# aconz2/font-ocr

Measured on AMD Instinct MI355X. Metric: Mpixels/s scanned (95-glyph x --x-bits=2 bank), higher is better.
Workload: dtype i8

## Files before the change

font_ocr_amd/csrc/hip/post.hip:

```cpp
#include <cstring>

#include "common.h"

namespace focr {

__device__ __forceinline__ int32_t total_key(float f) {
    int32_t b = __float_as_int(f);
    return b ^ (int32_t)(((uint32_t)(b >> 31)) >> 1);
}

__global__ void mark_anchor_rows(const uint64_t *__restrict__ hkeys, const float *__restrict__ hsims, const uint8_t *__restrict__ keep,
                                 const uint64_t *__restrict__ n_p, uint64_t ub, KeyFmt fmt, float anchor, uint32_t r_h, uint8_t *__restrict__ keep_row,
                                 uint32_t *__restrict__ line_b, uint32_t *__restrict__ line_e) {
    size_t i = (size_t)blockIdx.x * blockDim.x + threadIdx.x;
    const size_t n = (size_t)min(*n_p, ub);
    if (i >= n) return;
    const uint64_t k = hkeys[i];
    const size_t row = (size_t)fmt.page(k) * r_h + fmt.y(k);
    if (i == 0 || fmt.line(hkeys[i - 1]) != fmt.line(k)) line_b[row] = (uint32_t)i;
    if (i + 1 == n || fmt.line(hkeys[i + 1]) != fmt.line(k)) line_e[row] = (uint32_t)(i + 1);
    if (keep[i] && hsims[i] >= anchor) keep_row[row] = 1;
}

__device__ __forceinline__ uint32_t wave_umax(uint32_t v) {
    v = max(v, (uint32_t)__builtin_amdgcn_update_dpp(0, (int)v, 0x111, 0xf, 0xf, true));
    v = max(v, (uint32_t)__builtin_amdgcn_update_dpp(0, (int)v, 0x112, 0xf, 0xf, true));
    v = max(v, (uint32_t)__builtin_amdgcn_update_dpp(0, (int)v, 0x114, 0xf, 0xf, true));
    v = max(v, (uint32_t)__builtin_amdgcn_update_dpp(0, (int)v, 0x118, 0xf, 0xf, true));
    v = max(v, (uint32_t)__builtin_amdgcn_update_dpp(0, (int)v, 0x142, 0xa, 0xf, true));
    v = max(v, (uint32_t)__builtin_amdgcn_update_dpp(0, (int)v, 0x143, 0xc, 0xf, true));
    return (uint32_t)__builtin_amdgcn_readlane((int)v, 63);
}

constexpr uint32_t WALK_ROWS = 16;

struct Top {
    uint32_t ord, idx, letter, t, x;
    bool has;
};
__device__ __forceinline__ bool top_beats(const Top &a, const Top &b) { return b.has && (!a.has || b.ord > a.ord || (b.ord == a.ord && b.idx > a.idx)); }
struct RunnerArgs {
    const uint32_t *t_letter;
    const uint64_t *scanned;
    focr_runner_t *out;
    uint32_t bound;
};
__device__ __forceinline__ void store_runner(const RunnerArgs &ra, uint32_t slot, uint32_t members, const Top &second) {
    if (slot >= ra.bound) return;
    focr_runner_t r;
    r.members = members;
    r.letter = r.template_index = FOCR_NO_RUNNER;
    r.similarity = -__builtin_inff();
    r.x = r.reserved = 0;
    if (second.has) {
        r.letter = second.letter;
        r.template_index = second.t;
        r.similarity = __int_as_float(total_key(__int_as_float((int32_t)(second.ord ^ 0x80000000u))));
        r.x = (uint16_t)second.x;
    }
    ra.out[slot] = r;
}

struct NoArgs {};
__device__ __forceinline__ NoArgs runner_args() { return {}; }
__device__ __forceinline__ const RunnerArgs &runner_args(const RunnerArgs &ra) { return ra; }
template <bool RUNNERS, typename... Extra>
__global__ __launch_bounds__(256) void walk_kernel(const uint64_t *__restrict__ keys, const float *__restrict__ sims,
                                                   const uint8_t *__restrict__ keep, KeyFmt fmt, uint32_t n_rows_total,
                                                   int32_t overlap, const uint8_t *__restrict__ keep_row,
                                                   const uint32_t *__restrict__ line_b, const uint32_t *__restrict__ line_e,
                                                   uint32_t *__restrict__ choice, uint64_t *__restrict__ row_groups,
                                                   const Extra... extra) {
    static_assert(sizeof...(Extra) == (RUNNERS ? 1 : 0), "walk_runners takes one RunnerArgs, walk_lines nothing");
    [[maybe_unused]] const auto ra = runner_args(extra...);
    const uint32_t wave_id = (blockIdx.x * blockDim.x + threadIdx.x) >> 6, lane = threadIdx.x & 63;
    const uint32_t row_first = wave_id * WALK_ROWS;
    if (row_first >= n_rows_total) return;
    const uint32_t my_row = row_first + lane;
    const bool mine = lane < WALK_ROWS && my_row < n_rows_total && keep_row[my_row] != 0;
    const uint32_t my_b = mine ? line_b[my_row] : 0u, my_e = mine ? line_e[my_row] : 0u;
    for (uint64_t todo = __builtin_amdgcn_ballot_w64(mine); todo; todo &= todo - 1) {
    const int src = (int)__builtin_ctzll(todo);
    const uint32_t wave = row_first + (uint32_t)src;
    const uint64_t b = (uint32_t)__builtin_amdgcn_readlane((int)my_b, src), e = (uint32_t)__builtin_amdgcn_readlane((int)my_e, src);

    uint32_t groups = 0;
    bool open = false;
    int32_t anchor = 0;
    uint32_t best_ord = 0, best_idx = 0;
    Top a1{}, a2{};
    uint32_t members = 0, slot0 = 0;
    if constexpr (RUNNERS) slot0 = (uint32_t)ra.scanned[wave];
    for (uint64_t base = b; base < e; base += 64) {
        const uint64_t i = base + lane;
        const bool valid = i < e && keep[i];
        const int32_t x = valid ? (int32_t)fmt.x(keys[i]) : 0x7fffffff;
        const uint32_t ord = valid ? ((uint32_t)total_key(sims[i]) ^ 0x80000000u) : 0u;
        uint32_t let = 0, tt = 0;
        if constexpr (RUNNERS) {
            tt = valid ? fmt.t(keys[i]) : 0u;
            let = valid ? ra.t_letter[tt] : 0u;
        }
        const uint64_t vmask = __builtin_amdgcn_ballot_w64(valid);
        uint32_t pos = 0;
        int32_t opened_at = -1;
        while (pos < 64) {
            if (!open) {
                const uint64_t cand = vmask & (~0ull << pos);
                if (!cand) break;
                pos = (uint32_t)__builtin_ctzll(cand);
                anchor = __builtin_amdgcn_readlane(x, (int)pos);
                opened_at = (int32_t)pos;
                best_ord = 0;
                best_idx = 0;
                open = true;
                if constexpr (RUNNERS) a1.has = a2.has = false, members = 0;
            }
            const bool in = valid && lane >= pos && ((int32_t)lane == opened_at || ((x - anchor <= overlap) && (anchor - x <= overlap)));
            const uint64_t inmask = __builtin_amdgcn_ballot_w64(in);
            const uint64_t brk = vmask & ~inmask & (~0ull << pos);
            const uint32_t stop = brk ? (uint32_t)__builtin_ctzll(brk) : 64u;
            const bool member = in && lane < stop;
            const uint32_t mx = wave_umax(member ? ord : 0u);
            const uint64_t top = __builtin_amdgcn_ballot_w64(member && ord == mx);
            if (top && mx >= best_ord) {
                best_ord = mx;
                best_idx = (uint32_t)(base - b) + (63u - (uint32_t)__builtin_clzll(top));
            }
            if constexpr (RUNNERS) {
                members += (uint32_t)__builtin_popcountll(__builtin_amdgcn_ballot_w64(member));
                if (top) {
                    const int l1 = 63 - (int)__builtin_clzll(top);
                    const Top m1{mx, (uint32_t)(base - b) + (uint32_t)l1, (uint32_t)__builtin_amdgcn_readlane((int)let, l1),
                                 (uint32_t)__builtin_amdgcn_readlane((int)tt, l1), (uint32_t)__builtin_amdgcn_readlane(x, l1), true};
                    Top m2{};
                    const bool other = member && let != m1.letter;
                    if (__builtin_amdgcn_ballot_w64(other)) {
                        const uint32_t mx2 = wave_umax(other ? ord : 0u);
                        const int l2 = 63 - (int)__builtin_clzll(__builtin_amdgcn_ballot_w64(other && ord == mx2));
                        m2 = Top{mx2, (uint32_t)(base - b) + (uint32_t)l2, (uint32_t)__builtin_amdgcn_readlane((int)let, l2),
                                 (uint32_t)__builtin_amdgcn_readlane((int)tt, l2), (uint32_t)__builtin_amdgcn_readlane(x, l2), true};
                    }
                    Top lose = m1;
                    if (!a1.has || m1.ord >= a1.ord) lose = a1, a1 = m1;
                    Top s{};
                    if (lose.has && lose.letter != a1.letter) s = lose;
                    if (a2.has && a2.letter != a1.letter && top_beats(s, a2)) s = a2;
                    if (m2.has && m2.letter != a1.letter && top_beats(s, m2)) s = m2;
                    a2 = s;
                }
            }
            if (stop < 64) {
                if constexpr (RUNNERS) {
                    if (lane == 0) store_runner(ra, slot0 + groups, members, a2);
                } else {
                    if (lane == 0) choice[b + groups] = (uint32_t)b + best_idx;
                }
                groups++;
                open = false;
            }
            pos = stop;
        }
    }
    if (open) {
        if constexpr (RUNNERS) {
            if (lane == 0) store_runner(ra, slot0 + groups, members, a2);
        } else {
            if (lane == 0) choice[b + groups] = (uint32_t)b + best_idx;
        }
        groups++;
    }
    if constexpr (!RUNNERS)
        if (lane == 0) row_groups[wave] = ((uint64_t)1 << 32) | groups;
    }
}

constexpr auto walk_lines = walk_kernel<false>;
constexpr auto walk_runners = walk_kernel<true, RunnerArgs>;

__global__ void emit_chars(const uint64_t *__restrict__ keys, const float *__restrict__ sims, const uint64_t *__restrict__ n_p, uint64_t ub, KeyFmt fmt, uint32_t r_h,
                           const uint8_t *__restrict__ keep_row, const uint32_t *__restrict__ line_b,
                           const uint32_t *__restrict__ choice, const uint64_t *__restrict__ row_groups,
                           const uint64_t *__restrict__ scanned, const uint32_t *__restrict__ t_w,
                           const uint32_t *__restrict__ t_h, const uint32_t *__restrict__ t_letter,
                           uint64_t *__restrict__ line_char_off, focr_hit_t *__restrict__ chars) {
    size_t i = (size_t)blockIdx.x * blockDim.x + threadIdx.x;
    if (i >= min(*n_p, ub)) return;
    const uint64_t ki = keys[i];
    const size_t row = (size_t)fmt.page(ki) * r_h + fmt.y(ki);
    if (!keep_row[row]) return;
    const uint32_t k = (uint32_t)i - line_b[row];
    if (k >= (uint32_t)row_groups[row]) return;
    const uint64_t sc = scanned[row];
    const uint64_t off = (sc & 0xffffffffu) + k;
    if (k == 0) line_char_off[sc >> 32] = sc & 0xffffffffu;
    const uint32_t e = choice[i];
    const uint64_t key = keys[e];
    const uint32_t t = fmt.t(key);
    focr_hit_t h;
    h.x = (uint16_t)fmt.x(key);
    h.y = (uint16_t)fmt.y(key);
    h.w = (uint16_t)t_w[t];
    h.h = (uint16_t)t_h[t];
    h.similarity = sims[e];
    h.letter = t_letter[t];
    h.template_index = t;
    chars[off] = h;
}

__global__ void page_offsets(const uint64_t *__restrict__ scanned, uint32_t r_h, uint32_t n_pages, uint64_t *__restrict__ page_line_off) {
    uint32_t p = blockIdx.x * blockDim.x + threadIdx.x;
    if (p > n_pages) return;
    page_line_off[p] = scanned[(size_t)min(p, n_pages) * r_h] >> 32;
}

__global__ __launch_bounds__(256) void copy_chars_kernel(const uint32_t *__restrict__ src, const uint64_t *__restrict__ total, uint32_t *__restrict__ dst, uint64_t dst_dwords) {
    constexpr uint64_t DW = sizeof(focr_hit_t) / 4;
    const uint64_t n = min((*total & 0xffffffffull) * DW, dst_dwords);
    for (uint64_t i = (uint64_t)blockIdx.x * blockDim.x + threadIdx.x; i < n; i += (uint64_t)gridDim.x * blockDim.x) dst[i] = src[i];
}

bool post_queue_chars_copy(focr_ctx *c, void *dst, size_t dst_bytes) {
    static_assert(sizeof(focr_hit_t) % 4 == 0, "focr_hit_t is copied as dwords");
    if (!c->post_pending || !c->post_scanned.p || !c->post_chars.p || !dst) return false;
    const size_t n_rows_total = c->n_pages * c->pages.r_h;
    hipLaunchKernelGGL(copy_chars_kernel, dim3(64), dim3(256), 0, c->stream, (const uint32_t *)c->post_chars.p, (const uint64_t *)c->post_scanned.p + n_rows_total,
                       (uint32_t *)dst, (uint64_t)(dst_bytes / 4));
    return hipGetLastError() == hipSuccess;
}

}

using namespace focr;

extern "C" {

int focr_process_hits(focr_ctx_t *c, float anchor_threshold, int32_t overlap) {
    if (!c) return FOCR_ERR_INVALID;
    if (!c->scanned) return fail(c, FOCR_ERR_STATE, "focr_process_hits: no scan results");
    FOCR_HIP(c, hipSetDevice(c->device));
    c->post_starts();
    c->post_anchor = anchor_threshold;
    c->post_overlap = overlap;
    const size_t ub = c->ub_hits, n_pages = c->n_pages;
    if (!c->sizes_pending && (c->n_hits == 0 || c->n_matches == 0)) {
        c->processed = true;
        c->ms[MS_POST] = 0.f;
        return FOCR_OK;
    }
    if (ub >= 0xffffffffull) return fail(c, FOCR_ERR_OVERFLOW, "focr_process_hits: more than 2^32 hits in one batch");
    FOCR_HIP(c, hipEventRecord(c->ev[EV_POST_BEGIN], c->stream));
    const size_t n_rows_total = n_pages * c->pages.r_h;
    if (!c->scratch(c->post_keep, n_rows_total + 8) || !c->scratch(c->post_choice, ub + 1) || !c->scratch(c->post_packed, n_rows_total + 1) ||
        !c->scratch(c->post_scanned, n_rows_total + 1) || !c->scratch(c->post_page_off, n_pages + 1) || !c->scratch(c->post_line_be, 2 * n_rows_total) ||
        !c->scratch(c->post_line_off, n_rows_total + 1) || !c->scratch(c->post_chars, ub + 1))
        return fail(c, FOCR_ERR_NOMEM, "focr_process_hits: hipMalloc failed");
    uint8_t *keep_row = c->post_keep;
    uint32_t *choice = c->post_choice, *line_b = c->post_line_be, *line_e = line_b + n_rows_total;
    uint64_t *packed = c->post_packed, *scanned = c->post_scanned;
    uint64_t *d_page_off = c->post_page_off, *d_line_off = c->post_line_off;
    focr_hit_t *d_chars = c->post_chars;
    const uint8_t *keep = c->ord_keep;
    {
        ClearList clear{};
        if (!clear.add(keep_row, n_rows_total)) return fail(c, FOCR_ERR_INVALID, "focr_process_hits: clear list full or region too large");
        if (!clear.add(packed, (n_rows_total + 1) * 8)) return fail(c, FOCR_ERR_INVALID, "focr_process_hits: clear list full or region too large");
        if (int rc = launch_clear(c, clear)) return rc;
    }
    const unsigned nb = (unsigned)((ub + 255) / 256);
    if (ub)
        hipLaunchKernelGGL(mark_anchor_rows, dim3(nb), dim3(256), 0, c->stream, c->d_hkeys, c->d_hsims, keep, c->d_n_hits, (uint64_t)ub, c->fmt,
                           anchor_threshold, (uint32_t)c->pages.r_h, keep_row, line_b, line_e);
    hipLaunchKernelGGL(walk_lines, dim3((unsigned)(((n_rows_total + WALK_ROWS - 1) / WALK_ROWS * 64 + 255) / 256)), dim3(256), 0, c->stream, c->d_hkeys, c->d_hsims,
                       keep, c->fmt, (uint32_t)n_rows_total, overlap, keep_row, line_b, line_e, choice, packed);
    int rc;
    if ((rc = exclusive_scan_u64(c, packed, scanned, n_rows_total + 1))) return rc;
    FOCR_HIP(c, hipMemcpyAsync(&c->h_res->lines_chars, scanned + n_rows_total, sizeof(uint64_t), hipMemcpyDeviceToHost, c->stream));
    if (ub)
        hipLaunchKernelGGL(emit_chars, dim3(nb), dim3(256), 0, c->stream, c->d_hkeys, c->d_hsims, c->d_n_hits, (uint64_t)ub, c->fmt, (uint32_t)c->pages.r_h,
                           keep_row, line_b, choice, packed, scanned, c->bank.d_t_w, c->bank.d_t_h, c->bank.d_t_letter, d_line_off, d_chars);
    hipLaunchKernelGGL(page_offsets, dim3((unsigned)((n_pages + 1 + 255) / 256)), dim3(256), 0, c->stream, scanned, (uint32_t)c->pages.r_h,
                       (uint32_t)n_pages, d_page_off);
    FOCR_HIP(c, hipGetLastError());
    FOCR_HIP(c, hipEventRecord(c->ev[EV_POST_END], c->stream));
    c->post_pending = true;
    c->processed = true;
    if (!c->sizes_pending) return finish_results(c);
    return FOCR_OK;
}

static int fetch_lines(focr_ctx *c) {
    int rc0 = finish_results(c);
    if (rc0) return rc0;
    if (c->lines_on_host) return FOCR_OK;
    c->h_page_line_off.assign(c->n_pages + 1, 0);
    c->h_line_char_off.assign(c->n_lines + 1, 0);
    c->h_chars.resize(c->n_chars);
    if (c->n_matches && (c->n_lines || c->n_chars)) {
        FOCR_HIP(c, hipSetDevice(c->device));
        if (c->n_lines)
            FOCR_HIP(c, hipMemcpyAsync(c->h_line_char_off.data(), c->post_line_off.p, c->n_lines * 8, hipMemcpyDeviceToHost, c->io_stream));
        FOCR_HIP(c, hipMemcpyAsync(c->h_page_line_off.data(), c->post_page_off.p, (c->n_pages + 1) * 8, hipMemcpyDeviceToHost, c->io_stream));
        if (c->n_chars)
            FOCR_HIP(c, hipMemcpyAsync(c->h_chars.data(), c->post_chars.p, c->n_chars * sizeof(focr_hit_t), hipMemcpyDeviceToHost, c->io_stream));
        FOCR_HIP(c, hipStreamSynchronize(c->io_stream));
    }
    c->h_line_char_off[c->n_lines] = c->n_chars;
    c->lines_on_host = true;
    return FOCR_OK;
}

size_t focr_total_chars(focr_ctx_t *c) { return (c && c->processed && finish_results(c) == FOCR_OK) ? c->n_chars : 0; }
size_t focr_total_lines(focr_ctx_t *c) { return (c && c->processed && finish_results(c) == FOCR_OK) ? c->n_lines : 0; }

int focr_get_lines(focr_ctx_t *c, uint64_t *page_line_offsets, uint64_t *line_char_offsets, focr_hit_t *chars) {
    if (!c) return FOCR_ERR_INVALID;
    if (!c->processed) return fail(c, FOCR_ERR_STATE, "focr_get_lines: call focr_process_hits first");
    int rc = fetch_lines(c);
    if (rc) return rc;
    if (page_line_offsets) memcpy(page_line_offsets, c->h_page_line_off.data(), c->h_page_line_off.size() * 8);
    if (line_char_offsets) memcpy(line_char_offsets, c->h_line_char_off.data(), c->h_line_char_off.size() * 8);
    if (chars && c->n_chars) memcpy(chars, c->h_chars.data(), c->n_chars * sizeof(focr_hit_t));
    return FOCR_OK;
}

int focr_get_lines_into(focr_ctx_t *c, uint64_t *page_line_offsets, uint64_t *line_char_offsets, focr_hit_t *chars) {
    if (!c || !page_line_offsets || !line_char_offsets || !chars) return FOCR_ERR_INVALID;
    if (!c->processed) return fail(c, FOCR_ERR_STATE, "focr_get_lines_into: call focr_process_hits first");
    int rc = finish_results(c);
    if (rc) return rc;
    FOCR_HIP(c, hipSetDevice(c->device));
    if (c->n_matches && (c->n_lines || c->n_chars)) {
        if (c->n_lines) FOCR_HIP(c, hipMemcpyAsync(line_char_offsets, c->post_line_off.p, c->n_lines * 8, hipMemcpyDeviceToHost, c->io_stream));
        FOCR_HIP(c, hipMemcpyAsync(page_line_offsets, c->post_page_off.p, (c->n_pages + 1) * 8, hipMemcpyDeviceToHost, c->io_stream));
        if (c->n_chars) FOCR_HIP(c, hipMemcpyAsync(chars, c->post_chars.p, c->n_chars * sizeof(focr_hit_t), hipMemcpyDeviceToHost, c->io_stream));
        FOCR_HIP(c, hipStreamSynchronize(c->io_stream));
    } else {
        for (size_t p = 0; p <= c->n_pages; p++) page_line_offsets[p] = 0;
    }
    line_char_offsets[c->n_lines] = c->n_chars;
    return FOCR_OK;
}

const focr_hit_t *focr_lines_device_chars(focr_ctx_t *c) {
    return (c && c->processed && finish_results(c) == FOCR_OK && c->n_chars) ? (const focr_hit_t *)c->post_chars.p : nullptr;
}

int focr_get_runners(focr_ctx_t *c, focr_runner_t *out) {
    if (!c) return FOCR_ERR_INVALID;
    c->run_ms = 0.f;
    c->run_launches = 0;
    if (!c->scanned || !c->processed) return fail(c, FOCR_ERR_STATE, "focr_get_runners: call focr_process_hits first (after the last scan)");
    if (int rc = finish_results(c)) return rc;
    const size_t n_chars = c->n_chars;
    if (!n_chars) return FOCR_OK;
    if (!out) return fail(c, FOCR_ERR_INVALID, "focr_get_runners: no output buffer");
    FOCR_HIP(c, hipSetDevice(c->device));
    const hipStream_t s = c->io_stream;
    if (!c->runners_valid) {
        const size_t bound = c->ub_hits + 1, n_rows_total = c->n_pages * c->pages.r_h;
        if (bound >= 0xffffffffull) return fail(c, FOCR_ERR_OVERFLOW, "focr_get_runners: more than 2^32 hits in one batch");
        if (c->post_runners.reserve(bound, Grow::quarter, nullptr) != hipSuccess) return fail(c, FOCR_ERR_NOMEM, "focr_get_runners: hipMalloc failed");
        FOCR_HIP(c, hipEventRecord(c->run_ev[0], s));
        hipLaunchKernelGGL(walk_runners, dim3((unsigned)(((n_rows_total + WALK_ROWS - 1) / WALK_ROWS * 64 + 255) / 256)), dim3(256), 0, s, (const uint64_t *)c->d_hkeys,
                           (const float *)c->d_hsims, (const uint8_t *)c->ord_keep.p, c->fmt, (uint32_t)n_rows_total, c->post_overlap, (const uint8_t *)c->post_keep.p,
                           (const uint32_t *)c->post_line_be.p, (const uint32_t *)c->post_line_be.p + n_rows_total, (uint32_t *)nullptr, (uint64_t *)nullptr,
                           RunnerArgs{c->bank.d_t_letter.p, c->post_scanned.p, c->post_runners.p, (uint32_t)bound});
        FOCR_HIP(c, hipGetLastError());
        FOCR_HIP(c, hipEventRecord(c->run_ev[1], s));
    }
    FOCR_HIP(c, hipMemcpyAsync(out, c->post_runners.p, n_chars * sizeof(focr_runner_t), hipMemcpyDeviceToHost, s));
    FOCR_HIP(c, hipStreamSynchronize(s));
    if (!c->runners_valid) {
        FOCR_HIP(c, hipEventElapsedTime(&c->run_ms, c->run_ev[0], c->run_ev[1]));
        c->run_launches = 1;
        c->runners_valid = true;
    }
    return FOCR_OK;
}

int focr_last_runners(focr_ctx_t *c, float *ms, uint32_t *launches) {
    if (!c) return FOCR_ERR_INVALID;
    if (ms) *ms = c->run_ms;
    if (launches) *launches = c->run_launches;
    return FOCR_OK;
}

int focr_debug_process_hits(focr_ctx_t *c, const uint32_t *page, const uint32_t *y, const uint32_t *x, const uint32_t *t,
                            const float *similarity, const uint8_t *keep, size_t n) {
    if (!c) return FOCR_ERR_INVALID;
    if (n && (!page || !y || !x || !t || !similarity || !keep)) return fail(c, FOCR_ERR_INVALID, "focr_debug_process_hits: bad arguments");
    if (!c->n_templates || !c->pages.u8) return fail(c, FOCR_ERR_STATE, "focr_debug_process_hits: upload a bank and allocate pages first");
    if (n >= 0xffffffffull) return fail(c, FOCR_ERR_OVERFLOW, "focr_debug_process_hits: more than 2^32 hits in one batch");
    const KeyFmt fmt = key_format(c->n_templates, c->pages.r_w, c->pages.r_h, c->n_pages);
    std::vector<uint64_t> keys(n);
    std::vector<uint8_t> kept(n);
    size_t n_kept = 0;
    for (size_t i = 0; i < n; i++) {
        if (page[i] >= c->n_pages || y[i] >= c->pages.r_h || x[i] >= c->pages.r_w || t[i] >= c->n_templates)
            return fail(c, FOCR_ERR_INVALID, "focr_debug_process_hits: hit " + std::to_string(i) + " lies outside the pages or the bank");
        keys[i] = fmt.pack(page[i], y[i], x[i], t[i]);
        if (i && keys[i] <= keys[i - 1])
            return fail(c, FOCR_ERR_INVALID, "focr_debug_process_hits: hit " + std::to_string(i) + " does not follow its predecessor in (page, y, x, t)");
        kept[i] = keep[i] != 0;
        n_kept += kept[i];
    }
    if (int rc = finish_results(c)) return rc;
    FOCR_HIP(c, hipSetDevice(c->device));
    if (!c->scratch(c->acc_hkeys, n + 1) || !c->scratch(c->acc_hsims, n + 1) || !c->scratch(c->ord_keep, n + 1))
        return fail(c, FOCR_ERR_NOMEM, "focr_debug_process_hits: hipMalloc failed");
    uint64_t *d_keys = c->acc_hkeys;
    float *d_sims = c->acc_hsims;
    uint8_t *d_keep = c->ord_keep;
    if (n) {
        FOCR_HIP(c, hipMemcpyAsync(d_keys, keys.data(), n * 8, hipMemcpyHostToDevice, c->stream));
        FOCR_HIP(c, hipMemcpyAsync(d_sims, similarity, n * 4, hipMemcpyHostToDevice, c->stream));
        FOCR_HIP(c, hipMemcpyAsync(d_keep, kept.data(), n, hipMemcpyHostToDevice, c->stream));
    }
    if (int rc = install_host_hits(c, n)) return rc;
    FOCR_HIP(c, hipStreamSynchronize(c->stream));
    c->fmt = fmt;
    c->d_hkeys = d_keys;
    c->d_hsims = d_sims;
    c->n_hits = c->n_hits_raw = n;
    c->n_matches = n_kept;
    c->sub_p0 = 0;
    c->sub_np = c->n_pages;
    c->estimated = false;
    c->debug_hits_installed();
    return FOCR_OK;
}

}
```

Baseline: 34200.

## Fuse anchor marking into row walk with binary search and parallel chunk walk

Drops the clear launch and the per-hit mark_anchor_rows kernel. A new walk_rows kernel binary-searches the sorted keys to find each 16-row window's hit range, computes line begin/end, the anchor flags and zeroed row_groups itself, then walks each row 64 hits at a time using wave-parallel jump pointers and segmented max scans instead of a serial scan. emit_chars becomes a row-parallel emit_rows kernel. This saves launches and memory passes over all hits, but the walk logic is much more intricate, which raises the risk of subtle grouping mismatches.

```diff
diff --git a/font_ocr_amd/csrc/hip/post.hip b/font_ocr_amd/csrc/hip/post.hip
--- a/font_ocr_amd/csrc/hip/post.hip
+++ b/font_ocr_amd/csrc/hip/post.hip
@@ -7,19 +7,6 @@
 __device__ __forceinline__ int32_t total_key(float f) {
     int32_t b = __float_as_int(f);
     return b ^ (int32_t)(((uint32_t)(b >> 31)) >> 1);
-}
-
-__global__ void mark_anchor_rows(const uint64_t *__restrict__ hkeys, const float *__restrict__ hsims, const uint8_t *__restrict__ keep,
-                                 const uint64_t *__restrict__ n_p, uint64_t ub, KeyFmt fmt, float anchor, uint32_t r_h, uint8_t *__restrict__ keep_row,
-                                 uint32_t *__restrict__ line_b, uint32_t *__restrict__ line_e) {
-    size_t i = (size_t)blockIdx.x * blockDim.x + threadIdx.x;
-    const size_t n = (size_t)min(*n_p, ub);
-    if (i >= n) return;
-    const uint64_t k = hkeys[i];
-    const size_t row = (size_t)fmt.page(k) * r_h + fmt.y(k);
-    if (i == 0 || fmt.line(hkeys[i - 1]) != fmt.line(k)) line_b[row] = (uint32_t)i;
-    if (i + 1 == n || fmt.line(hkeys[i + 1]) != fmt.line(k)) line_e[row] = (uint32_t)(i + 1);
-    if (keep[i] && hsims[i] >= anchor) keep_row[row] = 1;
 }
 
 __device__ __forceinline__ uint32_t wave_umax(uint32_t v) {
@@ -30,6 +17,107 @@
     v = max(v, (uint32_t)__builtin_amdgcn_update_dpp(0, (int)v, 0x142, 0xa, 0xf, true));
     v = max(v, (uint32_t)__builtin_amdgcn_update_dpp(0, (int)v, 0x143, 0xc, 0xf, true));
     return (uint32_t)__builtin_amdgcn_readlane((int)v, 63);
+}
+
+__device__ __forceinline__ uint32_t lane_pull(uint32_t v, uint32_t src_lane) {
+    return (uint32_t)__builtin_amdgcn_ds_bpermute((int)(src_lane << 2), (int)v);
+}
+__device__ __forceinline__ uint32_t top_bit(uint64_t m) { return m ? 63u - (uint32_t)__builtin_clzll(m) : 0u; }
+__device__ __forceinline__ uint64_t bits_below(uint32_t n) { return n < 64 ? (1ull << n) - 1 : ~0ull; }
+
+__device__ __forceinline__ uint32_t walk_row_chunks(const uint64_t *__restrict__ keys, const float *__restrict__ sims, const uint8_t *__restrict__ keep,
+                                                    const KeyFmt fmt, const uint64_t b, const uint64_t e, const int32_t overlap,
+                                                    uint32_t *__restrict__ choice, const uint32_t lane) {
+    uint32_t groups = 0;
+    bool open = false;
+    int32_t anchor = 0;
+    uint32_t best_ord = 0, best_idx = 0;
+    for (uint64_t base = b; base < e; base += 64) {
+        const uint64_t i = base + lane;
+        const bool inrow = i < e, valid = inrow && keep[i];
+        const int32_t x = inrow ? (int32_t)fmt.x(keys[i]) : 0x7fffffff;
+        const uint32_t ord = valid ? ((uint32_t)total_key(sims[i]) ^ 0x80000000u) : 0u;
+        const uint64_t vmask = __builtin_amdgcn_ballot_w64(valid);
+        if (!vmask) continue;
+        uint32_t head;
+        if (open && overlap >= 0) {
+            const uint64_t out = __builtin_amdgcn_ballot_w64(valid && x - anchor > overlap);
+            head = out ? (uint32_t)__builtin_ctzll(out) : 64u;
+        } else {
+            head = (uint32_t)__builtin_ctzll(vmask);
+        }
+        uint32_t s0 = 0, s1 = head, succ = 64;
+        if (head < 64) {
+            uint32_t j0 = lane + 1;
+            if (overlap >= 0) {
+                uint32_t pos = 0;
+#pragma unroll
+                for (uint32_t step = 32; step; step >>= 1) {
+                    const int32_t xp = (int32_t)lane_pull((uint32_t)x, pos + step);
+                    if (!(xp - x > overlap)) pos += step;
+                }
+                j0 = pos + 1;
+            }
+            const uint64_t rest = j0 < 64 ? vmask >> j0 : 0ull;
+            succ = rest ? j0 + (uint32_t)__builtin_ctzll(rest) : 64u;
+            uint32_t jump[6];
+            jump[0] = succ;
+#pragma unroll
+            for (int k = 1; k < 6; k++) {
+                const uint32_t t = lane_pull(jump[k - 1], jump[k - 1]);
+                jump[k] = jump[k - 1] < 64 ? t : 64u;
+            }
+            uint32_t cur = head;
+#pragma unroll
+            for (int k = 5; k >= 0; k--) {
+                const uint32_t nxt = lane_pull(jump[k], cur);
+                if (nxt <= lane) cur = nxt;
+            }
+            const uint32_t cur_end = lane_pull(succ, cur);
+            if (lane >= head) s0 = cur, s1 = cur_end;
+        }
+        uint32_t pm = ord;
+#pragma unroll
+        for (uint32_t d = 1; d < 64; d <<= 1) {
+            const uint32_t o = lane_pull(pm, lane - d);
+            if (lane >= s0 + d) pm = max(pm, o);
+        }
+        const uint32_t smax = lane_pull(pm, s1 - 1);
+        const uint64_t tops = __builtin_amdgcn_ballot_w64(valid && ord == smax);
+        if (open) {
+            const uint64_t top = tops & bits_below(head);
+            if (top) {
+                const uint32_t mx = (uint32_t)__builtin_amdgcn_readlane((int)pm, (int)head - 1);
+                if (mx >= best_ord) {
+                    best_ord = mx;
+                    best_idx = (uint32_t)(base - b) + top_bit(top);
+                }
+            }
+            if (head < 64) {
+                if (lane == 0) choice[b + groups] = (uint32_t)b + best_idx;
+                groups++;
+                open = false;
+            }
+        }
+        if (head < 64) {
+            const bool opener = lane >= head && s0 == lane;
+            const uint64_t openers = __builtin_amdgcn_ballot_w64(opener);
+            const uint32_t win = top_bit(tops & ~bits_below(lane) & bits_below(succ));
+            const uint32_t gid = (uint32_t)__builtin_popcountll(openers & bits_below(lane));
+            if (opener && succ < 64) choice[b + groups + gid] = (uint32_t)base + win;
+            const int last = (int)top_bit(openers);
+            open = true;
+            anchor = __builtin_amdgcn_readlane(x, last);
+            best_ord = (uint32_t)__builtin_amdgcn_readlane((int)smax, last);
+            best_idx = (uint32_t)(base - b) + (uint32_t)__builtin_amdgcn_readlane((int)win, last);
+            groups += (uint32_t)__builtin_popcountll(openers) - 1;
+        }
+    }
+    if (open) {
+        if (lane == 0) choice[b + groups] = (uint32_t)b + best_idx;
+        groups++;
+    }
+    return groups;
 }
 
 constexpr uint32_t WALK_ROWS = 16;
@@ -71,7 +159,7 @@
                                                    const uint32_t *__restrict__ line_b, const uint32_t *__restrict__ line_e,
                                                    uint32_t *__restrict__ choice, uint64_t *__restrict__ row_groups,
                                                    const Extra... extra) {
-    static_assert(sizeof...(Extra) == (RUNNERS ? 1 : 0), "walk_runners takes one RunnerArgs, walk_lines nothing");
+    static_assert(sizeof...(Extra) == (RUNNERS ? 1 : 0), "walk_runners takes one RunnerArgs");
     [[maybe_unused]] const auto ra = runner_args(extra...);
     const uint32_t wave_id = (blockIdx.x * blockDim.x + threadIdx.x) >> 6, lane = threadIdx.x & 63;
     const uint32_t row_first = wave_id * WALK_ROWS;
@@ -175,37 +263,116 @@
     }
 }
 
-constexpr auto walk_lines = walk_kernel<false>;
+
+__device__ __forceinline__ uint32_t wave_or(uint32_t v) {
+    v |= (uint32_t)__builtin_amdgcn_update_dpp(0, (int)v, 0x111, 0xf, 0xf, true);
+    v |= (uint32_t)__builtin_amdgcn_update_dpp(0, (int)v, 0x112, 0xf, 0xf, true);
+    v |= (uint32_t)__builtin_amdgcn_update_dpp(0, (int)v, 0x114, 0xf, 0xf, true);
+    v |= (uint32_t)__builtin_amdgcn_update_dpp(0, (int)v, 0x118, 0xf, 0xf, true);
+    v |= (uint32_t)__builtin_amdgcn_update_dpp(0, (int)v, 0x142, 0xa, 0xf, true);
+    v |= (uint32_t)__builtin_amdgcn_update_dpp(0, (int)v, 0x143, 0xc, 0xf, true);
+    return (uint32_t)__builtin_amdgcn_readlane((int)v, 63);
+}
+
+__global__ __launch_bounds__(256) void walk_rows(const uint64_t *__restrict__ keys, const float *__restrict__ sims, const uint8_t *__restrict__ keep,
+                                                 const uint64_t *__restrict__ n_p, uint64_t ub, KeyFmt fmt, uint32_t r_h, uint32_t n_rows_total, float anchor_thr,
+                                                 int32_t overlap, uint8_t *__restrict__ keep_row, uint32_t *__restrict__ line_b, uint32_t *__restrict__ line_e,
+                                                 uint32_t *__restrict__ choice, uint64_t *__restrict__ row_groups) {
+    const uint32_t wave_id = (blockIdx.x * blockDim.x + threadIdx.x) >> 6, lane = threadIdx.x & 63;
+    const uint32_t row_first = wave_id * WALK_ROWS;
+    if (wave_id == 0 && lane == 0) row_groups[n_rows_total] = 0;
+    if (row_first >= n_rows_total) return;
+    const uint32_t n = (uint32_t)min(*n_p, ub);
+    const uint32_t my_row = row_first + lane;
+    const uint32_t half = lane >> 5, sub = lane & 31;
+    const uint32_t t_row = row_first + half * WALK_ROWS, t_page = t_row / r_h;
+    const uint64_t t_line = ((uint64_t)t_page << fmt.by) | (t_row - t_page * r_h);
+    uint32_t lo = t_row < n_rows_total ? 0u : n, hi = n;
+    while (__builtin_amdgcn_ballot_w64(hi - lo > 32)) {
+        const bool wide = hi - lo > 32;
+        const uint32_t step = (hi - lo) >> 5, q = lo + sub * step + (step - 1);
+        const uint64_t below = __builtin_amdgcn_ballot_w64(wide && fmt.line(keys[wide ? q : 0u]) < t_line);
+        const uint32_t c = (uint32_t)__builtin_popcount((uint32_t)(below >> (32 * half)));
+        if (wide) {
+            if (c < 32) hi = lo + c * step + (step - 1);
+            lo += c * step;
+        }
+    }
+    {
+        const uint32_t q = lo + sub;
+        const uint64_t below = __builtin_amdgcn_ballot_w64(q < hi && fmt.line(keys[q < hi ? q : 0u]) < t_line);
+        lo += (uint32_t)__builtin_popcount((uint32_t)(below >> (32 * half)));
+    }
+    const uint32_t first = (uint32_t)__builtin_amdgcn_readlane((int)lo, 0), last = (uint32_t)__builtin_amdgcn_readlane((int)lo, 32);
+    uint32_t seen = 0;
+    uint32_t rows_below[WALK_ROWS - 1] = {};
+    for (uint64_t base = first; base < last; base += 64) {
+        const uint64_t i = base + lane;
+        uint32_t r = WALK_ROWS;
+        if (i < last) {
+            const uint64_t k = keys[i];
+            r = fmt.page(k) * r_h + fmt.y(k) - row_first;
+            if (r < WALK_ROWS && keep[i] && sims[i] >= anchor_thr) seen |= 1u << r;
+        }
+#pragma unroll
+        for (uint32_t j = 0; j < WALK_ROWS - 1; j++) rows_below[j] += (uint32_t)__builtin_popcountll(__builtin_amdgcn_ballot_w64(r <= j));
+    }
+    seen = wave_or(seen);
+    uint32_t my_b = lane < WALK_ROWS ? first : last;
+#pragma unroll
+    for (uint32_t j = 0; j < WALK_ROWS - 1; j++)
+        if (lane == j + 1) my_b = first + rows_below[j];
+    const uint32_t my_e = lane_pull(my_b, lane + 1);
+    const bool owned = lane < WALK_ROWS && my_row < n_rows_total;
+    if (owned) {
+        keep_row[my_row] = (uint8_t)((seen >> lane) & 1u);
+        line_b[my_row] = my_b;
+        line_e[my_row] = my_e;
+        if (!((seen >> lane) & 1u)) row_groups[my_row] = 0;
+    }
+    for (uint32_t todo = seen; todo; todo &= todo - 1) {
+        const int src = __builtin_ctz(todo);
+        const uint64_t b = (uint32_t)__builtin_amdgcn_readlane((int)my_b, src), e = (uint32_t)__builtin_amdgcn_readlane((int)my_e, src);
+        const uint32_t groups = walk_row_chunks(keys, sims, keep, fmt, b, e, overlap, choice, lane);
+        if (lane == 0) row_groups[row_first + (uint32_t)src] = ((uint64_t)1 << 32) | groups;
+    }
+}
+
 constexpr auto walk_runners = walk_kernel<true, RunnerArgs>;
 
-__global__ void emit_chars(const uint64_t *__restrict__ keys, const float *__restrict__ sims, const uint64_t *__restrict__ n_p, uint64_t ub, KeyFmt fmt, uint32_t r_h,
-                           const uint8_t *__restrict__ keep_row, const uint32_t *__restrict__ line_b,
-                           const uint32_t *__restrict__ choice, const uint64_t *__restrict__ row_groups,
-                           const uint64_t *__restrict__ scanned, const uint32_t *__restrict__ t_w,
-                           const uint32_t *__restrict__ t_h, const uint32_t *__restrict__ t_letter,
-                           uint64_t *__restrict__ line_char_off, focr_hit_t *__restrict__ chars) {
-    size_t i = (size_t)blockIdx.x * blockDim.x + threadIdx.x;
-    if (i >= min(*n_p, ub)) return;
-    const uint64_t ki = keys[i];
-    const size_t row = (size_t)fmt.page(ki) * r_h + fmt.y(ki);
-    if (!keep_row[row]) return;
-    const uint32_t k = (uint32_t)i - line_b[row];
-    if (k >= (uint32_t)row_groups[row]) return;
-    const uint64_t sc = scanned[row];
-    const uint64_t off = (sc & 0xffffffffu) + k;
-    if (k == 0) line_char_off[sc >> 32] = sc & 0xffffffffu;
-    const uint32_t e = choice[i];
-    const uint64_t key = keys[e];
-    const uint32_t t = fmt.t(key);
-    focr_hit_t h;
-    h.x = (uint16_t)fmt.x(key);
-    h.y = (uint16_t)fmt.y(key);
-    h.w = (uint16_t)t_w[t];
-    h.h = (uint16_t)t_h[t];
-    h.similarity = sims[e];
-    h.letter = t_letter[t];
-    h.template_index = t;
-    chars[off] = h;
+__global__ __launch_bounds__(256) void emit_rows(const uint64_t *__restrict__ keys, const float *__restrict__ sims, KeyFmt fmt, uint32_t n_rows_total,
+                                                 const uint8_t *__restrict__ keep_row, const uint32_t *__restrict__ line_b,
+                                                 const uint32_t *__restrict__ choice, const uint64_t *__restrict__ row_groups,
+                                                 const uint64_t *__restrict__ scanned, const uint32_t *__restrict__ t_w,
+                                                 const uint32_t *__restrict__ t_h, const uint32_t *__restrict__ t_letter,
+                                                 uint64_t *__restrict__ line_char_off, focr_hit_t *__restrict__ chars) {
+    const uint32_t wave_id = (blockIdx.x * blockDim.x + threadIdx.x) >> 6, lane = threadIdx.x & 63;
+    const uint32_t row_first = wave_id * WALK_ROWS;
+    if (row_first >= n_rows_total) return;
+    const uint32_t my_row = row_first + lane;
+    const bool mine = lane < WALK_ROWS && my_row < n_rows_total && keep_row[my_row] != 0;
+    const uint32_t my_b = mine ? line_b[my_row] : 0u, my_groups = mine ? (uint32_t)row_groups[my_row] : 0u;
+    const uint64_t my_sc = mine ? scanned[my_row] : 0ull;
+    if (mine) line_char_off[my_sc >> 32] = my_sc & 0xffffffffu;
+    for (uint64_t todo = __builtin_amdgcn_ballot_w64(mine); todo; todo &= todo - 1) {
+        const int src = (int)__builtin_ctzll(todo);
+        const uint32_t b = (uint32_t)__builtin_amdgcn_readlane((int)my_b, src), groups = (uint32_t)__builtin_amdgcn_readlane((int)my_groups, src);
+        const uint32_t first = (uint32_t)__builtin_amdgcn_readlane((int)(uint32_t)my_sc, src);
+        for (uint32_t k = lane; k < groups; k += 64) {
+            const uint32_t e = choice[(uint64_t)b + k];
+            const uint64_t key = keys[e];
+            const uint32_t t = fmt.t(key);
+            focr_hit_t h;
+            h.x = (uint16_t)fmt.x(key);
+            h.y = (uint16_t)fmt.y(key);
+            h.w = (uint16_t)t_w[t];
+            h.h = (uint16_t)t_h[t];
+            h.similarity = sims[e];
+            h.letter = t_letter[t];
+            h.template_index = t;
+            chars[(uint64_t)first + k] = h;
+        }
+    }
 }
 
 __global__ void page_offsets(const uint64_t *__restrict__ scanned, uint32_t r_h, uint32_t n_pages, uint64_t *__restrict__ page_line_off) {
@@ -261,24 +428,14 @@
     uint64_t *d_page_off = c->post_page_off, *d_line_off = c->post_line_off;
     focr_hit_t *d_chars = c->post_chars;
     const uint8_t *keep = c->ord_keep;
-    {
-        ClearList clear{};
-        if (!clear.add(keep_row, n_rows_total)) return fail(c, FOCR_ERR_INVALID, "focr_process_hits: clear list full or region too large");
-        if (!clear.add(packed, (n_rows_total + 1) * 8)) return fail(c, FOCR_ERR_INVALID, "focr_process_hits: clear list full or region too large");
-        if (int rc = launch_clear(c, clear)) return rc;
-    }
-    const unsigned nb = (unsigned)((ub + 255) / 256);
-    if (ub)
-        hipLaunchKernelGGL(mark_anchor_rows, dim3(nb), dim3(256), 0, c->stream, c->d_hkeys, c->d_hsims, keep, c->d_n_hits, (uint64_t)ub, c->fmt,
-                           anchor_threshold, (uint32_t)c->pages.r_h, keep_row, line_b, line_e);
-    hipLaunchKernelGGL(walk_lines, dim3((unsigned)(((n_rows_total + WALK_ROWS - 1) / WALK_ROWS * 64 + 255) / 256)), dim3(256), 0, c->stream, c->d_hkeys, c->d_hsims,
-                       keep, c->fmt, (uint32_t)n_rows_total, overlap, keep_row, line_b, line_e, choice, packed);
+    const unsigned row_blocks = (unsigned)(((n_rows_total + WALK_ROWS - 1) / WALK_ROWS * 64 + 255) / 256);
+    hipLaunchKernelGGL(walk_rows, dim3(row_blocks), dim3(256), 0, c->stream, c->d_hkeys, c->d_hsims, keep, c->d_n_hits, (uint64_t)ub, c->fmt, (uint32_t)c->pages.r_h,
+                       (uint32_t)n_rows_total, anchor_threshold, overlap, keep_row, line_b, line_e, choice, packed);
     int rc;
     if ((rc = exclusive_scan_u64(c, packed, scanned, n_rows_total + 1))) return rc;
     FOCR_HIP(c, hipMemcpyAsync(&c->h_res->lines_chars, scanned + n_rows_total, sizeof(uint64_t), hipMemcpyDeviceToHost, c->stream));
-    if (ub)
-        hipLaunchKernelGGL(emit_chars, dim3(nb), dim3(256), 0, c->stream, c->d_hkeys, c->d_hsims, c->d_n_hits, (uint64_t)ub, c->fmt, (uint32_t)c->pages.r_h,
-                           keep_row, line_b, choice, packed, scanned, c->bank.d_t_w, c->bank.d_t_h, c->bank.d_t_letter, d_line_off, d_chars);
+    hipLaunchKernelGGL(emit_rows, dim3(row_blocks), dim3(256), 0, c->stream, c->d_hkeys, c->d_hsims, c->fmt, (uint32_t)n_rows_total, keep_row, line_b, choice, packed,
+                       scanned, c->bank.d_t_w, c->bank.d_t_h, c->bank.d_t_letter, d_line_off, d_chars);
     hipLaunchKernelGGL(page_offsets, dim3((unsigned)((n_pages + 1 + 255) / 256)), dim3(256), 0, c->stream, scanned, (uint32_t)c->pages.r_h,
                        (uint32_t)n_pages, d_page_off);
     FOCR_HIP(c, hipGetLastError());
```

Result: no change. 34350 (median of 6 runs) (+0.5%).
